# alexfrom0815/IR-BPP

Hardware: AMD Instinct MI355X
Metric: env steps/sec (placements/sec) across N parallel bins (higher is better)
Workload: dtype f64

## Files before the change

irbpp_amd/build.py:

```python
from __future__ import annotations

import os
import shutil
import subprocess

PKG_DIR = os.path.dirname(os.path.abspath(__file__))
CSRC = os.path.join(PKG_DIR, "csrc")
LIB_PATH = os.path.join(PKG_DIR, "libirbpp_hip.so")
SOURCES = ["irbpp_capi.hip", "irbpp_kernels.hip", "irbpp_wide.hip", "irbpp_replay.hip", "irbpp_replay_pool.hip", "irbpp_metrics.hip", "irbpp_metrics.h", "irbpp_device.h", "contours_device.h", "irbpp_itemgen.h",
           "irbpp_itemgen.hip", "irbpp_itemgen_device.h", "irbpp_rotalias.h", "irbpp_head.h", "irbpp_c51.hip", "irbpp_dueling.hip", "irbpp_dueling_loss.hip", "irbpp_streams.hip", "irbpp_plan.h", "irbpp_binstate.h", "irbpp_binstate.hip",
           os.path.join("..", "..", "include", "irbpp.h")]
HIPCC_FLAGS = ["--offload-arch=gfx950", "-O3", "-std=c++17", "-ffp-contract=off", "-fno-honor-nans",
               "-shared", "-fPIC", "-Wno-unused-value"]


def source_hash() -> str:
    import hashlib
    h = hashlib.sha256(" ".join(HIPCC_FLAGS).encode())
    for name in sorted(SOURCES):
        with open(os.path.join(CSRC, name), "rb") as f:
            h.update(f.read())
    return h.hexdigest()[:16]


def _hipcc() -> str:
    for cand in (shutil.which("hipcc"), "/opt/rocm/bin/hipcc"):
        if cand and os.path.exists(cand):
            return cand
    raise RuntimeError("hipcc not found: the HIP library cannot be built on this machine")


def built_hash(path: str = LIB_PATH) -> str:
    try:
        with open(path, "rb") as f:
            blob = f.read()
    except OSError:
        return ""
    i = blob.find(b"irbpp-source-hash:")
    return blob[i + 18:i + 34].decode("ascii", "replace") if i >= 0 else ""


def needs_build(path: str = LIB_PATH) -> bool:
    return built_hash(path) != source_hash()


def build(force: bool = False, verbose: bool = False) -> str:
    out = LIB_PATH
    if not force and not needs_build(out):
        return out
    cmd = [_hipcc()] + HIPCC_FLAGS + [f'-DIRBPP_SOURCE_HASH="{source_hash()}"', os.path.join(CSRC, "irbpp_capi.hip"), "-o", out]
    if verbose:
        print(" ".join(cmd))
    res = subprocess.run(cmd, capture_output=True, text=True)
    if res.returncode != 0:
        raise RuntimeError("hipcc failed:\n" + res.stdout + res.stderr)
    from . import asmcheck
    try:
        chk = asmcheck.check_library(out)
    except (RuntimeError, OSError, subprocess.CalledProcessError) as e:
        if verbose:
            print(f"asmcheck skipped: {e}")
        return out
    if verbose:
        print(f"asmcheck: {chk['scalar_loads']} scalar loads in {chk['functions']} kernels, {len(chk['problems'])} hazards")
    if chk["problems"]:
        os.replace(out, out + ".rejected")
        raise RuntimeError("scalar-load hazard in the built library (kept as " + out + ".rejected):\n" + "\n".join(chk["problems"]))
    return out
```

irbpp_amd/csrc/irbpp_kernels.hip:

```cpp
#include <hip/hip_runtime.h>
#include <math.h>
#include <stdint.h>

#include "contours_device.h"
#include "irbpp_device.h"
#include "../../include/irbpp.h"

#ifndef IRBPP_PASS
#define IRBPP_PASS 1
#endif

#undef IRBPP_HERE
#undef IRBPP_PASS_NS
#if IRBPP_PASS == 1
#define IRBPP_HERE ::irbpp::
#elif IRBPP_PASS == 2
#define IRBPP_HERE ::irbpp::wg512::
#define IRBPP_PASS_NS wg512
#else
#define IRBPP_HERE ::irbpp::wg128::
#define IRBPP_PASS_NS wg128
#endif

namespace irbpp {
#if IRBPP_PASS != 1
namespace IRBPP_PASS_NS {
#endif

#if IRBPP_PASS == 1
constexpr int BLOCK = 256;
#elif IRBPP_PASS == 2
constexpr int BLOCK = 512;
#else
constexpr int BLOCK = 128;
#endif
constexpr int WAVES = BLOCK / 64;

#ifndef IRBPP_REPS
#ifdef IRBPP_ABLATE
#define IRBPP_REPS(bit) (1 + ((P.dbg_repeat >> (bit)) & 1))
#else
#define IRBPP_REPS(bit) 1
#endif
#endif

#if IRBPP_PASS == 1
__device__ __forceinline__ double round6(double x) { return rint(x * 1e6) / 1e6; }

__device__ __forceinline__ double round6_scaled(double x) { return rint(x * 1e6); }

__device__ __forceinline__ int np_floor_divide_int(double a, double b, double inv_b) {
    const double x = fabs(a);
    const double q0 = trunc(x * inv_b);
    const double r0 = fma(-q0, b, x);
    int q = (int)q0 + (r0 >= b ? 1 : 0) - (r0 < 0.0 ? 1 : 0);
#if defined(__HIP_DEVICE_COMPILE__)
    if (__ballot(a < 0.0) == 0ull) return q;
#endif
    if (a < 0.0) {
        const double r = fma(-(double)q, b, x);
        q = r == 0.0 ? -q : -q - 1;
    }
    return q;
}

template <int CTRL, int ROW_MASK>
__device__ __forceinline__ int dpp_shift(int v) { return __builtin_amdgcn_update_dpp(0, v, CTRL, ROW_MASK, 0xF, false); }
__device__ __forceinline__ int wave_inclusive_sum(int v) {
    v += dpp_shift<0x111, 0xF>(v);
    v += dpp_shift<0x112, 0xF>(v);
    v += dpp_shift<0x114, 0xF>(v);
    v += dpp_shift<0x118, 0xF>(v);
    v += dpp_shift<0x142, 0xA>(v);
    v += dpp_shift<0x143, 0xC>(v);
    return v;
}
__device__ __forceinline__ int imax(int a, int b) { return a > b ? a : b; }
__device__ __forceinline__ int wave_inclusive_max(int v) {
    v = imax(v, dpp_shift<0x111, 0xF>(v));
    v = imax(v, dpp_shift<0x112, 0xF>(v));
    v = imax(v, dpp_shift<0x114, 0xF>(v));
    v = imax(v, dpp_shift<0x118, 0xF>(v));
    v = imax(v, dpp_shift<0x142, 0xA>(v));
    v = imax(v, dpp_shift<0x143, 0xC>(v));
    return v;
}

__device__ __forceinline__ double wave_max_f64(double v) {
#define IRBPP_MAX_STEP(CTRL, ROWS)                                                                                   \
    {                                                                                                                \
        const int lo = __builtin_amdgcn_update_dpp(__double2loint(v), __double2loint(v), CTRL, ROWS, 0xF, false);    \
        const int hi = __builtin_amdgcn_update_dpp(__double2hiint(v), __double2hiint(v), CTRL, ROWS, 0xF, false);    \
        v = fmax(v, __hiloint2double(hi, lo));                                                                       \
    }
    IRBPP_MAX_STEP(0x111, 0xF) IRBPP_MAX_STEP(0x112, 0xF) IRBPP_MAX_STEP(0x114, 0xF) IRBPP_MAX_STEP(0x118, 0xF)
    IRBPP_MAX_STEP(0x142, 0xA) IRBPP_MAX_STEP(0x143, 0xC)
#undef IRBPP_MAX_STEP
    return __hiloint2double(__builtin_amdgcn_readlane(__double2hiint(v), 63), __builtin_amdgcn_readlane(__double2loint(v), 63));
}

#endif
__device__ inline double block_max_f64(double v, double* red) {
    v = wave_max_f64(v);
    __syncthreads();
    if ((threadIdx.x & 63) == 0) red[threadIdx.x >> 6] = v;
    __syncthreads();
    double r = red[0];
    for (int w = 1; w < WAVES; ++w) r = fmax(r, red[w]);
    return r;
}

__device__ inline int block_sum_int(int v, int* red) {
    v = __builtin_amdgcn_readlane(wave_inclusive_sum(v), 63);
    __syncthreads();
    if ((threadIdx.x & 63) == 0) red[threadIdx.x >> 6] = v;
    __syncthreads();
    int r = 0;
    for (int w = 0; w < WAVES; ++w) r += red[w];
    return r;
}

__device__ inline int block_scan_flag(bool flag, int* red, int& total) {
    const unsigned long long bal = __ballot(flag);
    const int lane = threadIdx.x & 63, w = threadIdx.x >> 6;
    const int pre = __popcll(bal & ((1ull << lane) - 1ull));
    __syncthreads();
    if (lane == 0) red[w] = __popcll(bal);
    __syncthreads();
    int base = 0;
    total = 0;
    for (int i = 0; i < WAVES; ++i) {
        const int c = red[i];
        if (i < w) base += c;
        total += c;
    }
    return base + pre;
}

#if IRBPP_PASS == 1
__device__ inline int trajectory_row(const Params& P, const Tables& T, int b, int episode) {
    long long row = T.stream ? (long long)b : (long long)P.traj_start + P.goff + b + (long long)episode * P.gbins;
    row %= T.n_traj;
    if (row < 0) row += T.n_traj;
    return (int)row;
}
struct KernArgs;
__device__ __forceinline__ void raise_error(const State& S, int bit);
constexpr int STREAM_CONSUMED = -3;
__device__ inline int consume_item(const Tables& T, const State& S, int row, int cursor, int id) {
    if (T.stream) {
        if (id == STREAM_CONSUMED) { raise_error(S, IRBPP_DEVERR_STREAM_DRY); return -1; }
        const_cast<int32_t*>(T.seq)[(long long)row * T.seq_len + (int)((uint32_t)cursor % (uint32_t)T.seq_len)] = STREAM_CONSUMED;
    }
    if (id >= T.n_shapes) { raise_error(S, IRBPP_DEVERR_BAD_ITEM); return -1; }
    return id < 0 ? -1 : id;
}
__device__ inline int fetch_item(const Tables& T, const State& S, int row, int cursor) {
    if (!T.stream && cursor >= T.seq_len) return -1;
    const int at = T.stream ? (int)((uint32_t)cursor % (uint32_t)T.seq_len) : cursor;
    return consume_item(T, S, row, cursor, T.seq[(long long)row * T.seq_len + at]);
}

__device__ __forceinline__ int fdiv(int n, int d, uint32_t m) {
    return d == 1 ? n : (int)__umulhi((uint32_t)n, m);
}

struct KernArgs { Params P; Tables T; State S; StepIO io; int mode; };
typedef const __attribute__((address_space(4))) KernArgs* KernArgsPtr;
__device__ __forceinline__ KernArgsPtr cold_args() {
// ... 1496 lines not shown
                    } else {
                        k = keys[row];
                    }
                    float rv;
                    if (fallback) rv = (float)((gvalid[(k >> 16) * 16 + ((k >> 8) & 255u)] >> (k & 255u)) & 1u);
                    else rv = (float)zsrc[(k >> 16) * AC + ((k >> 8) & 255u) * Ay + (k & 255u)];
                    v0 = (float)(k >> 16);
                    v1 = (float)((k >> 8) & 255u);
                    v2 = (float)(k & 255u);
                    v3 = fallback ? (float)P.bin_z : rv;
                    v4 = fallback ? rv : 1.0f;
                    S.cand[(size_t)b * P.S + row] = k;
                    if (!fallback && rv < best) { best = rv; bi = row; }
                }
                float* const o = obs + 5 * row;
                o[0] = v0; o[1] = v1; o[2] = v2; o[3] = v3; o[4] = v4;
            }
            if (lane == 0) {
                S.bs[b].cur_item = item;
                S.bs[b].nvalid = nvalid;
                S.bs[b].nrows = nrows;
            }
            if (io.auto_action != nullptr) {
#define IRBPP_ARGMIN_STEP(CTRL, ROWS)                                                                                          \
                {                                                                                                              \
                    const float ob = __int_as_float(__builtin_amdgcn_update_dpp(__float_as_int(best), __float_as_int(best), CTRL, ROWS, 0xF, false)); \
                    const int oi = __builtin_amdgcn_update_dpp(bi, bi, CTRL, ROWS, 0xF, false);                                 \
                    if (ob < best || (ob == best && oi < bi)) { best = ob; bi = oi; }                                           \
                }
                IRBPP_ARGMIN_STEP(0x111, 0xF) IRBPP_ARGMIN_STEP(0x112, 0xF) IRBPP_ARGMIN_STEP(0x114, 0xF) IRBPP_ARGMIN_STEP(0x118, 0xF)
                IRBPP_ARGMIN_STEP(0x142, 0xA) IRBPP_ARGMIN_STEP(0x143, 0xC)
#undef IRBPP_ARGMIN_STEP
                if (lane == 63) io.auto_action[b] = bi == 0x7fffffff ? 0 : bi;
            }
            stamp(io, b, 4, lane == 0);
        }
    }
    __syncthreads();
    if ((need[0] & need[1] & need[2] & need[3]) == -1) return;
    Lds L = {};
    L.vmask = (uint32_t*)(smem + P.e_vmask);
    L.redd = (double*)(smem + P.e_red);
    L.redi = (int*)(L.redd + 8);
    L.img = (uint16_t*)(smem + P.e_hist);
    L.scratch = smem + P.e_keys;
#pragma unroll 1
    for (int w = 0; w < WAVES; ++w) {
        const int bw = __builtin_amdgcn_readfirstlane(need[w]);
        if (bw < 0) continue;
        const int slot_w = (int)blockIdx.x * WAVES + w + io.block_off;
        float* const obs = io.obs + (size_t)(some ? slot_w : bw) * io.obs_stride;
        const uint32_t* gv = S.w_vmask + (size_t)bw * R * 16;
        __syncthreads();
#pragma unroll 1
        for (int i = tid; i < R * 16; i += BLOCK) L.vmask[i] = gv[i];
        const int nvalid = S.w_meta[(size_t)bw * WMETA + 2], item = S.w_meta[(size_t)bw * WMETA + 3];
        const uint32_t amap_w = (uint32_t)S.w_meta[(size_t)bw * WMETA + 5];
        __syncthreads();
        stamp(io, bw, 3);
        emit_observation(P, S, io, L, bw, item, nvalid, obs, S.w_posz + (size_t)bw * R * AC, S.w_valid + (size_t)bw * R * 16, amap_w);
    }
}
#define IRBPP_EMIT_WAVE_KERNEL(NAME, SPEC)                                                                                  \
    extern "C" __global__ void __launch_bounds__(BLOCK) __attribute__((amdgpu_waves_per_eu(8, 8)))                      \
    NAME(const Params P, const Tables T, const State S, const StepIO io, const int mode) {                              \
        extern __shared__ __attribute__((aligned(16))) unsigned char smem[];                                            \
        emit_wave_body<SPEC>(P, T, S, io, mode, smem);                                                                  \
    }
IRBPP_EMIT_WAVE_KERNEL(irbpp_emit_wave_kernel, 0)
#ifndef IRBPP_NO_SPEC
IRBPP_EMIT_WAVE_KERNEL(irbpp_emit_wave_kernel_s1, 1)
IRBPP_EMIT_WAVE_KERNEL(irbpp_emit_wave_kernel_s2, 2)
IRBPP_EMIT_WAVE_KERNEL(irbpp_emit_wave_kernel_s5, 5)
#endif

#ifndef IRBPP_TRACE_SHORT
#define IRBPP_TRACE_SHORT 0
#endif
constexpr int TRACE_P = IRBPP_TRACE_P;
constexpr int TRACE_CAP = 128;
constexpr int TRACE_LDS_CAP = 56, TRACE_SLOT = TRACE_LDS_CAP + 4;
constexpr int TRACE_SPILL = TRACE_CAP - TRACE_LDS_CAP;
constexpr int TRACE_SHORT = IRBPP_TRACE_SHORT;
static_assert(TRACE_CAP <= 64 * TRACE_P, "a border must fit one polygon round");
static_assert(ROUND_POINTS == 64 * TRACE_P, "a round record holds one polygon round");
constexpr int TRACE_BIG = 768;
constexpr int TRACE_FSTRIDE = FRAME_WORDS;
static_assert(TRACE_FSTRIDE % 2 == 1 && (TRACE_SLOT / 4) % 2 == 1 && TRACE_SLOT % 4 == 0, "odd dword strides in LDS");
constexpr int TRACE_BIG_BYTES = 6 * TRACE_BIG + 64;
constexpr int TRACE_WAVE_BYTES = TRACE_BIG_BYTES + 64 * TRACE_SPILL;
template <int TRACE_CPW>
__device__ __forceinline__ void trace_body(const Params& P, const State& S, long long* prof) {
    constexpr int SLOT = TRACE_SLOT, CAP = TRACE_CAP, LCAP = TRACE_LDS_CAP, PP = TRACE_P;
    __shared__ __attribute__((aligned(16))) uint8_t slots[TRACE_CPW * SLOT];
    __shared__ __attribute__((aligned(16))) uint32_t sfr[TRACE_CPW * TRACE_FSTRIDE];
    __shared__ uint32_t dps[64 * PP];
    __shared__ uint8_t dpscratch[64 * PP];
    const int lane = threadIdx.x;
    const int seg_cap = P.seg_cap;
    int seg_n[NXCD], seg_first[NXCD + 1];
    seg_first[0] = 0;
#pragma unroll
    for (int s = 0; s < NXCD; ++s) {
        const int n = S.w_total[s * XCD_STRIDE];
        seg_n[s] = n < seg_cap ? n : seg_cap;
        seg_first[s + 1] = seg_first[s] + (seg_n[s] + TRACE_CPW - 1) / TRACE_CPW;
    }
    for (int chunk = blockIdx.x; chunk < seg_first[NXCD]; chunk += gridDim.x) {
        const long long t_start = prof ? (long long)clock64() : 0;
        int seg = 0;
#pragma unroll
        for (int s = 1; s < NXCD; ++s) seg += chunk >= seg_first[s] ? 1 : 0;
        int first_chunk = 0, count = 0;
#pragma unroll
        for (int s = 0; s < NXCD; ++s) if (s == seg) { first_chunk = seg_first[s]; count = seg_n[s]; }
        const int gi = (chunk - first_chunk) * TRACE_CPW + lane;
        const bool have = lane < TRACE_CPW && gi < count;
        const size_t g = (size_t)seg * seg_cap + gi;
        int my_n = 0, rk = 0, x0 = 0, y0 = 0;
        uint32_t* const fr = sfr + (lane < TRACE_CPW ? lane : 0) * TRACE_FSTRIDE;
        uint8_t* const my_slot = slots + (lane < TRACE_CPW ? lane : 0) * SLOT;
        uint8_t* const wave_spill = S.w_big + (size_t)blockIdx.x * TRACE_WAVE_BYTES + TRACE_BIG_BYTES;
        if (have) {
            const uint2 ce = S.w_cand[g];
            const uint32_t e = ce.y;
            const int b = (int)ce.x, img = (int)((e >> 8) & 511u);
            x0 = e & 15u;
            y0 = (e >> 4) & 15u;
            rk = b * P.R + (int)S.w_imgrot[(size_t)b * P.wimg + img];
            const uint4* gi = (const uint4*)(S.w_img + ((size_t)b * P.wimg + img) * 16);
            const uint4 v0 = gi[0], v1 = gi[1];
            const uint32_t w[8] = {v0.x, v0.y, v0.z, v0.w, v1.x, v1.y, v1.z, v1.w};
            uint32_t r[16], c[16];
#pragma unroll
            for (int q = 0; q < 8; ++q) {
                r[2 * q] = c[2 * q] = w[q] & 0xFFFFu;
                r[2 * q + 1] = c[2 * q + 1] = w[q] >> 16;
            }
            transpose16(c);
            frames_store(fr, r, c);
        }
        const long long t_staged = prof ? (long long)clock64() : 0;
        {
            const int n = trace_border_fast(fr, x0, y0, my_slot, LCAP, have, wave_spill + lane * TRACE_SPILL, TRACE_SPILL);
            if (n < 0) { if (lane == 0) atomicOr(S.err, IRBPP_DEVERR_TRACE_GUARD); }
            else my_n = n;
        }
        {
            unsigned long long big = __ballot(my_n > CAP);
            while (big != 0ull) {
                const int l0 = __ffsll((long long)big) - 1;
                big &= big - 1ull;
                if (lane == l0) {
                    uint8_t* gsc = S.w_big + (size_t)blockIdx.x * TRACE_WAVE_BYTES;
                    SlotMem m;
                    m.pts = gsc; m.dst = gsc + TRACE_BIG; m.stk = (uint32_t*)(gsc + 2 * TRACE_BIG); m.cap = TRACE_BIG; m.cap_stk = TRACE_BIG;
                    uint16_t* im = (uint16_t*)(gsc + 6 * TRACE_BIG);
                    for (int q = 0; q < 16; ++q) { im[q] = (uint16_t)frame_raw_row(fr, q); im[16 + q] = (uint16_t)frame_raw_col(fr, q); }
                    if (contour_vertices(im, im + 16, x0, y0, m, S.w_vmask + (size_t)rk * 16) != 0)
                        atomicOr(S.err, IRBPP_DEVERR_TRACE_GUARD);
                    my_n = 0;
                }
            }
        }
        const bool spilled = __ballot(my_n > LCAP) != 0ull;
        if (spilled) {
            __builtin_amdgcn_fence(__ATOMIC_RELEASE, "workgroup");
            __builtin_amdgcn_fence(__ATOMIC_ACQUIRE, "workgroup");
        }
        const long long t_traced = prof ? (long long)clock64() : 0;
        auto next_round = [&](int cls, int left, int& wn, int& excl, int& base) -> unsigned long long {
            wn = (cls == 0 ? left <= TRACE_SHORT : true) ? left : 0;
            const int incl = wave_inclusive_sum(wn);
            excl = incl - wn;
            if (__builtin_amdgcn_readlane(incl, 63) == 0) return 0ull;
            const unsigned long long todo = __ballot(wn > 0);
            base = __builtin_amdgcn_readlane(excl, __ffsll((long long)todo) - 1);
            return __ballot(wn > 0 && incl - base <= 64 * PP);
        };
        int n_rounds = 0;
        {
            int left = my_n;
            for (int cls = 0; cls < 2; ++cls)
                for (;;) {
                    int wn, excl, base = 0;
                    const unsigned long long sel = next_round(cls, left, wn, excl, base);
                    if (sel == 0ull) break;
                    if ((sel >> lane) & 1ull) left = 0;
                    ++n_rounds;
                }
        }
        const int round_cap = P.round_cap;
        const int xcd = (int)(__builtin_amdgcn_s_getreg((31 << 11) | 20) & (NXCD - 1));
        int at = 0;
        if (n_rounds > 0) {
            if (lane == 0) at = atomicAdd(S.w_nround + xcd * XCD_STRIDE, n_rounds);
            at = __builtin_amdgcn_readfirstlane(at);
        }
        const bool inline_dp = at + n_rounds > round_cap;
        uint8_t* const rec0 = S.w_round + ((size_t)xcd * round_cap + at) * ROUND_BYTES;
        int left = my_n, n_dp = 0;
        for (int cls = 0; cls < 2; ++cls)
        for (;;) {
            int wn, excl, base = 0;
            const unsigned long long sel = next_round(cls, left, wn, excl, base);
            if (sel == 0ull) break;
#pragma unroll
            for (int u = 0; u < PP; ++u) dps[u * 64 + lane] = 0u;
            IRBPP_WAVE_SYNC();
            if ((sel >> lane) & 1ull) dps[excl - base] = (uint32_t)lane + 1u;
            IRBPP_WAVE_SYNC();
            int mark[PP];
#pragma unroll
            for (int u = 0; u < PP; ++u) mark[u] = (int)dps[u * 64 + lane];
            IRBPP_WAVE_SYNC();
            bool live[PP];
            int pv[PP], jj[PP], nn[PP], sbq[PP], prk[PP];
            const uint8_t* pts[PP];
            int carry = 0;
#pragma unroll
            for (int u = 0; u < PP; ++u) {
                const int run = imax(wave_inclusive_max(mark[u]), carry);
                carry = __builtin_amdgcn_readlane(run, 63);
                const int owner = run - 1;
                const int on = owner >= 0 ? owner : 0;
                const int ns = __shfl(wn | ((excl - base) << 8), on);
                nn[u] = ns & 255;
                sbq[u] = ns >> 8;
                prk[u] = __shfl(rk, on);
                live[u] = owner >= 0 && u * 64 + lane < sbq[u] + nn[u];
                pts[u] = slots + on * SLOT;
                jj[u] = u * 64 + lane - sbq[u];
                if (!live[u]) { nn[u] = 1; sbq[u] = 0; jj[u] = 0; }
                pv[u] = live[u] ? (int)pts[u][jj[u] < LCAP ? jj[u] : LCAP] : 0;
                if (spilled && live[u] && jj[u] >= LCAP) pv[u] = (int)wave_spill[on * TRACE_SPILL + jj[u] - LCAP];
            }
            if (inline_dp) {
                approx_convex_segmented<PP>(lane, live, pv, jj, nn, sbq, pts, prk, dps, dpscratch, S.w_vmask);
            } else {
                uint8_t* const rec = rec0 + (size_t)n_dp * ROUND_BYTES;
#pragma unroll
                for (int u = 0; u < PP; ++u) {
                    const int q = u * 64 + lane;
                    rec[q] = (uint8_t)pv[u];
                    rec[64 * PP + q] = (uint8_t)(live[u] ? nn[u] : 0);
                    rec[2 * 64 * PP + q] = (uint8_t)sbq[u];
                    ((uint32_t*)(rec + 3 * 64 * PP))[q] = (uint32_t)prk[u];
                }
            }
            if ((sel >> lane) & 1ull) left = 0;
            ++n_dp;
        }
        if (inline_dp && n_rounds > 0 && at < round_cap) {
            const int lim = at + n_rounds < round_cap ? n_rounds : round_cap - at;
            for (int i = 0; i < lim; ++i)
#pragma unroll
                for (int u = 0; u < PP; ++u) rec0[(size_t)i * ROUND_BYTES + 64 * PP + u * 64 + lane] = 0;
        }
#if defined(IRBPP_AB_POLY_ACCOUNT) || defined(IRBPP_AB_EMIT_ACCOUNT)
        if (false) {
#else
        if (prof && lane == 0) {
#endif
            const int b0 = (int)S.w_cand[(size_t)seg * seg_cap + (size_t)(chunk - first_chunk) * TRACE_CPW].x;
            long long* row = prof + (size_t)b0 * PHASE_ROW;
            const long long t_end = (long long)clock64();
            row[11] = t_end - t_start;
            row[12] = t_staged - t_start;
            row[13] = t_traced - t_staged;
            row[14] = t_end - t_traced;
            row[15] = 1 | ((long long)n_dp << 20) | ((long long)(count - (chunk - first_chunk) * TRACE_CPW < TRACE_CPW ? count - (chunk - first_chunk) * TRACE_CPW : TRACE_CPW) << 40);
        }
        IRBPP_WAVE_SYNC();
    }
}

constexpr int TRACE_REFILL_BATCH = 128, TRACE_REFILL_THR = 32;
template <int BATCH, int THR>
__device__ __forceinline__ void trace_refill_body(const Params& P, const State& S, long long* prof) {
    constexpr int SLOT = TRACE_SLOT, CAP = TRACE_CAP, LCAP = TRACE_LDS_CAP, PP = TRACE_P, NCE = BATCH / 64;
    static_assert(BATCH % 64 == 0 && NCE >= 1 && NCE <= 4, "a batch is a whole number of wave-wide candidate loads");
    __shared__ __attribute__((aligned(16))) uint8_t slots[64 * SLOT];
    __shared__ __attribute__((aligned(16))) uint32_t sfr[64 * TRACE_FSTRIDE];
    __shared__ uint32_t dps[64 * PP];
    __shared__ uint8_t dpscratch[64 * PP];
    const int lane = threadIdx.x;
    const int seg_cap = P.seg_cap;
    int seg_n[NXCD], seg_first[NXCD + 1];
    seg_first[0] = 0;
#pragma unroll
    for (int s = 0; s < NXCD; ++s) {
        const int n = S.w_total[s * XCD_STRIDE];
        seg_n[s] = n < seg_cap ? n : seg_cap;
        seg_first[s + 1] = seg_first[s] + (seg_n[s] + BATCH - 1) / BATCH;
    }
    uint32_t* const fr = sfr + lane * TRACE_FSTRIDE;
    uint8_t* const my_slot = slots + lane * SLOT;
    uint8_t* const wave_spill = S.w_big + (size_t)blockIdx.x * TRACE_WAVE_BYTES + TRACE_BIG_BYTES;
    uint8_t* const my_spill = wave_spill + lane * TRACE_SPILL;
    IRBPP_WALK_TABLES(WT)
    const int round_cap = P.round_cap;
    const int xcd = (int)(__builtin_amdgcn_s_getreg((31 << 11) | 20) & (NXCD - 1));
    for (int chunk = blockIdx.x; chunk < seg_first[NXCD]; chunk += gridDim.x) {
        const long long t_start = prof ? (long long)clock64() : 0;
        int seg = 0;
#pragma unroll
        for (int s = 1; s < NXCD; ++s) seg += chunk >= seg_first[s] ? 1 : 0;
        int first_chunk = 0, count = 0;
#pragma unroll
        for (int s = 0; s < NXCD; ++s) if (s == seg) { first_chunk = seg_first[s]; count = seg_n[s]; }
        const int gi0 = (chunk - first_chunk) * BATCH;
        const int nb = count - gi0 < BATCH ? count - gi0 : BATCH;
        const uint2* const cl = S.w_cand + (size_t)seg * seg_cap + gi0;
        uint2 ce[NCE];
#pragma unroll
        for (int u = 0; u < NCE; ++u) ce[u] = u * 64 + lane < nb ? cl[u * 64 + lane] : make_uint2(0u, 0u);
        Walk w;
        w.pos = w.n = w.result = w.pos0 = w.pos1 = 0;
        w.nb16 = w.k2 = w.prev = w.s_close = w.run = 0u;
        int rk = 0, x0 = 0, y0 = 0, nxt = 0, n_dp_total = 0, refills = 0;
        uint2 pf_e = make_uint2(0u, 0u);
        uint4 pf0 = make_uint4(0u, 0u, 0u, 0u), pf1 = pf0;
        uint32_t pf_rot = 0u;
        auto prefetch = [&]() {
            const int c = nxt + lane;
            uint2 e = make_uint2(0u, 0u);
#pragma unroll
            for (int u = 0; u < NCE; ++u) {
                const uint32_t ex = (uint32_t)__shfl((int)ce[u].x, c & 63), ey = (uint32_t)__shfl((int)ce[u].y, c & 63);
                if ((c >> 6) == u) e = make_uint2(ex, ey);
            }
            pf_e = e;
            if (c < nb) {
                const size_t at = (size_t)e.x * P.wimg + ((e.y >> 8) & 511u);
                pf_rot = S.w_imgrot[at];
                const uint4* gi = (const uint4*)(S.w_img + at * 16);
                pf0 = gi[0];
                pf1 = gi[1];
            }
        };
        auto flush = [&]() {
            int my_n = w.run == 0u ? w.result : 0;
            w.result = w.run == 0u ? 0 : w.result;
            if (__ballot(my_n != 0) == 0ull) return;
            {
                unsigned long long big = __ballot(my_n > CAP);
                while (big != 0ull) {
                    const int l0 = __ffsll((long long)big) - 1;
                    big &= big - 1ull;
                    if (lane == l0) {
                        uint8_t* gsc = S.w_big + (size_t)blockIdx.x * TRACE_WAVE_BYTES;
                        SlotMem m;
                        m.pts = gsc; m.dst = gsc + TRACE_BIG; m.stk = (uint32_t*)(gsc + 2 * TRACE_BIG); m.cap = TRACE_BIG; m.cap_stk = TRACE_BIG;
                        uint16_t* im = (uint16_t*)(gsc + 6 * TRACE_BIG);
                        for (int q = 0; q < 16; ++q) { im[q] = (uint16_t)frame_raw_row(fr, q); im[16 + q] = (uint16_t)frame_raw_col(fr, q); }
                        if (contour_vertices(im, im + 16, x0, y0, m, S.w_vmask + (size_t)rk * 16) != 0)
                            atomicOr(S.err, IRBPP_DEVERR_TRACE_GUARD);
                        my_n = 0;
                    }
                }
            }
            const bool spilled = __ballot(my_n > LCAP) != 0ull;
            if (spilled) {
                __builtin_amdgcn_fence(__ATOMIC_RELEASE, "workgroup");
                __builtin_amdgcn_fence(__ATOMIC_ACQUIRE, "workgroup");
            }
            auto next_round = [&](int left, int& wn, int& excl, int& base) -> unsigned long long {
                wn = left;
                const int incl = wave_inclusive_sum(wn);
                excl = incl - wn;
                if (__builtin_amdgcn_readlane(incl, 63) == 0) return 0ull;
                const unsigned long long todo = __ballot(wn > 0);
                base = __builtin_amdgcn_readlane(excl, __ffsll((long long)todo) - 1);
                return __ballot(wn > 0 && incl - base <= 64 * PP);
            };
            int n_rounds = 0;
            {
                int left = my_n;
                for (;;) {
                    int wn, excl, base = 0;
                    const unsigned long long sel = next_round(left, wn, excl, base);
                    if (sel == 0ull) break;
                    if ((sel >> lane) & 1ull) left = 0;
                    ++n_rounds;
                }
            }
            int at = 0;
            if (n_rounds > 0) {
                if (lane == 0) at = atomicAdd(S.w_nround + xcd * XCD_STRIDE, n_rounds);
                at = __builtin_amdgcn_readfirstlane(at);
            }
            const bool inline_dp = at + n_rounds > round_cap;
            uint8_t* const rec0 = S.w_round + ((size_t)xcd * round_cap + at) * ROUND_BYTES;
            int left = my_n, n_dp = 0;
            for (;;) {
                int wn, excl, base = 0;
                const unsigned long long sel = next_round(left, wn, excl, base);
                if (sel == 0ull) break;
#pragma unroll
                for (int u = 0; u < PP; ++u) dps[u * 64 + lane] = 0u;
                IRBPP_WAVE_SYNC();
                if ((sel >> lane) & 1ull) dps[excl - base] = (uint32_t)lane + 1u;
                IRBPP_WAVE_SYNC();
                int mark[PP];
#pragma unroll
                for (int u = 0; u < PP; ++u) mark[u] = (int)dps[u * 64 + lane];
                IRBPP_WAVE_SYNC();
                bool live[PP];
                int pv[PP], jj[PP], nn[PP], sbq[PP], prk[PP];
                const uint8_t* pts[PP];
                int carry = 0;
#pragma unroll
                for (int u = 0; u < PP; ++u) {
                    const int run = imax(wave_inclusive_max(mark[u]), carry);
                    carry = __builtin_amdgcn_readlane(run, 63);
                    const int owner = run - 1;
                    const int on = owner >= 0 ? owner : 0;
                    const int ns = __shfl(wn | ((excl - base) << 8), on);
                    nn[u] = ns & 255;
                    sbq[u] = ns >> 8;
                    prk[u] = __shfl(rk, on);
                    live[u] = owner >= 0 && u * 64 + lane < sbq[u] + nn[u];
                    pts[u] = slots + on * SLOT;
                    jj[u] = u * 64 + lane - sbq[u];
                    if (!live[u]) { nn[u] = 1; sbq[u] = 0; jj[u] = 0; }
                    pv[u] = live[u] ? (int)pts[u][jj[u] < LCAP ? jj[u] : LCAP] : 0;
                    if (spilled && live[u] && jj[u] >= LCAP) pv[u] = (int)wave_spill[on * TRACE_SPILL + jj[u] - LCAP];
                }
                if (inline_dp) {
                    approx_convex_segmented<PP>(lane, live, pv, jj, nn, sbq, pts, prk, dps, dpscratch, S.w_vmask);
                } else {
                    uint8_t* const rec = rec0 + (size_t)n_dp * ROUND_BYTES;
#pragma unroll
                    for (int u = 0; u < PP; ++u) {
                        const int q = u * 64 + lane;
                        rec[q] = (uint8_t)pv[u];
                        rec[64 * PP + q] = (uint8_t)(live[u] ? nn[u] : 0);
                        rec[2 * 64 * PP + q] = (uint8_t)sbq[u];
                        ((uint32_t*)(rec + 3 * 64 * PP))[q] = (uint32_t)prk[u];
                    }
                }
                if ((sel >> lane) & 1ull) left = 0;
                ++n_dp;
            }
            if (inline_dp && n_rounds > 0 && at < round_cap) {
                const int lim = at + n_rounds < round_cap ? n_rounds : round_cap - at;
                for (int i = 0; i < lim; ++i)
#pragma unroll
                    for (int u = 0; u < PP; ++u) rec0[(size_t)i * ROUND_BYTES + 64 * PP + u * 64 + lane] = 0;
            }
            n_dp_total += n_dp;
            IRBPP_WAVE_SYNC();
        };
        prefetch();
        int guard = 16384;
        for (;;) {
            const unsigned long long walking = __ballot(w.run != 0u);
            const int idle = 64 - __popcll(walking);
            if ((idle >= THR && nxt < nb) || walking == 0ull) {
                flush();
                if (nxt >= nb) break;
                const int rank = (int)__builtin_amdgcn_mbcnt_hi((uint32_t)(~walking >> 32), __builtin_amdgcn_mbcnt_lo((uint32_t)~walking, 0u));
                const bool take = w.run == 0u && nxt + rank < nb;
                const uint32_t ex = (uint32_t)__shfl((int)pf_e.x, rank), ey = (uint32_t)__shfl((int)pf_e.y, rank);
                const uint32_t rot = (uint32_t)__shfl((int)pf_rot, rank);
                uint32_t wd[8];
                wd[0] = (uint32_t)__shfl((int)pf0.x, rank); wd[1] = (uint32_t)__shfl((int)pf0.y, rank);
                wd[2] = (uint32_t)__shfl((int)pf0.z, rank); wd[3] = (uint32_t)__shfl((int)pf0.w, rank);
                wd[4] = (uint32_t)__shfl((int)pf1.x, rank); wd[5] = (uint32_t)__shfl((int)pf1.y, rank);
                wd[6] = (uint32_t)__shfl((int)pf1.z, rank); wd[7] = (uint32_t)__shfl((int)pf1.w, rank);
                if (take) {
                    x0 = (int)(ey & 15u);
                    y0 = (int)((ey >> 4) & 15u);
                    rk = (int)ex * P.R + (int)rot;
                    uint32_t r[16], c[16];
#pragma unroll
                    for (int q = 0; q < 8; ++q) {
                        r[2 * q] = c[2 * q] = wd[q] & 0xFFFFu;
                        r[2 * q + 1] = c[2 * q + 1] = wd[q] >> 16;
                    }
                    transpose16(c);
                    frames_store(fr, r, c);
                    walk_start(w, fr, x0, y0, my_slot, LCAP, true, WT);
                }
                nxt += idle < nb - nxt ? idle : nb - nxt;
                ++refills;
                if (nxt < nb) prefetch();
                continue;
            }
            if (w.run != 0u) walk_iter(w, fr, my_slot, LCAP, my_spill, TRACE_SPILL, WT);
            if (--guard == 0) { if (lane == 0) atomicOr(S.err, IRBPP_DEVERR_TRACE_GUARD); break; }
        }
        if (prof && lane == 0) {
            const int b0 = (int)cl[0].x;
            long long* row = prof + (size_t)b0 * PHASE_ROW;
            const long long t_end = (long long)clock64();
            row[11] = t_end - t_start;
            row[12] = 0;
            row[13] = t_end - t_start;
            row[14] = (long long)refills | ((long long)(16384 - guard) << 16);
            row[15] = 1 | ((long long)n_dp_total << 20) | ((long long)nb << 40);
        }
        IRBPP_WAVE_SYNC();
    }
}
extern "C" __global__ void __launch_bounds__(64) irbpp_trace_kernel_refill(const Params P, const State S, long long* prof) {
    trace_refill_body<TRACE_REFILL_BATCH, TRACE_REFILL_THR>(P, S, prof);
}

extern "C" __global__ void __launch_bounds__(64) irbpp_trace_kernel(const Params P, const State S, long long* prof) { trace_body<64>(P, S, prof); }
extern "C" __global__ void __launch_bounds__(64) irbpp_trace_kernel_c32(const Params P, const State S, long long* prof) { trace_body<32>(P, S, prof); }
extern "C" __global__ void __launch_bounds__(64) irbpp_trace_kernel_c16(const Params P, const State S, long long* prof) { trace_body<16>(P, S, prof); }

extern "C" __global__ void __launch_bounds__(64)
irbpp_polygon_kernel(const Params P, const State S
#ifdef IRBPP_AB_POLY_ACCOUNT
                     , long long* prof
#endif
                     ) {
    constexpr int PP = TRACE_P;
#ifdef IRBPP_AB_POLY_ACCOUNT
    long long acct[8] = {0, 0, 0, 0, 0, 0, 0, 0};
    long long* const ac = prof ? acct : nullptr;
    const long long t_begin = (long long)clock64(), w_begin = (long long)wall_clock64();
    long long t_first_loaded = 0, cyc_hops = 0, cyc_dp = 0, cyc_rank = 0, cyc_tail = 0, rounds_done = 0;
#endif
    __shared__ uint32_t dps[64 * PP];
    __shared__ uint8_t dpscratch[64 * PP];
    __shared__ __attribute__((aligned(16))) uint8_t lpts[64 * PP];
    const int lane = threadIdx.x;
    const int round_cap = P.round_cap;
    int seg_n[NXCD], seg_first[NXCD + 1];
    seg_first[0] = 0;
#pragma unroll
    for (int s = 0; s < NXCD; ++s) {
        const int n = S.w_nround[s * XCD_STRIDE];
        seg_n[s] = n < round_cap ? n : round_cap;
        seg_first[s + 1] = seg_first[s] + seg_n[s];
    }
    for (int rd = blockIdx.x; rd < seg_first[NXCD]; rd += gridDim.x) {
        int seg = 0;
#pragma unroll
        for (int s = 1; s < NXCD; ++s) seg += rd >= seg_first[s] ? 1 : 0;
        int first = 0;
#pragma unroll
        for (int s = 0; s < NXCD; ++s) if (s == seg) first = seg_first[s];
        const uint8_t* const rec = S.w_round + ((size_t)seg * round_cap + (rd - first)) * ROUND_BYTES;
        bool live[PP];
        int pv[PP], jj[PP], nn[PP], sbq[PP], prk[PP];
        const uint8_t* pts[PP];
#pragma unroll
        for (int u = 0; u < PP; ++u) {
            const int q = u * 64 + lane;
            pv[u] = rec[q];
            nn[u] = rec[64 * PP + q];
            sbq[u] = rec[2 * 64 * PP + q];
            prk[u] = (int)((const uint32_t*)(rec + 3 * 64 * PP))[q];
            lpts[q] = (uint8_t)pv[u];
        }
        IRBPP_WAVE_SYNC();
#pragma unroll
        for (int u = 0; u < PP; ++u) {
            live[u] = nn[u] > 0;
            jj[u] = u * 64 + lane - sbq[u];
            if (!live[u]) { nn[u] = 1; sbq[u] = 0; jj[u] = 0; pv[u] = 0; }
            pts[u] = lpts + sbq[u];
        }
#ifdef IRBPP_AB_POLY_ACCOUNT
        const long long t_in = (long long)clock64();
        if (rounds_done == 0) t_first_loaded = t_in - t_begin;
        acct[1] = acct[2] = acct[3] = 0;
        approx_convex_segmented<PP>(lane, live, pv, jj, nn, sbq, pts, prk, dps, dpscratch, S.w_vmask, ac);
        const long long t_out = (long long)clock64();
        cyc_hops += acct[1] - t_in; cyc_dp += acct[2] - acct[1]; cyc_rank += acct[3] - acct[2]; cyc_tail += t_out - acct[3];
        ++rounds_done;
#else
        approx_convex_segmented<PP>(lane, live, pv, jj, nn, sbq, pts, prk, dps, dpscratch, S.w_vmask);
#endif
        IRBPP_WAVE_SYNC();
    }
#ifdef IRBPP_AB_POLY_ACCOUNT
    if (prof && lane == 0 && (int)blockIdx.x < P.N) {
        long long* row = prof + (size_t)blockIdx.x * PHASE_ROW;
        row[11] = (long long)clock64() - t_begin;
        row[12] = t_first_loaded | (((long long)(__builtin_amdgcn_s_getreg((31 << 11) | 20) & (NXCD - 1))) << 32);
        row[10] = w_begin;
        row[9] = (long long)wall_clock64();
        row[13] = cyc_hops | (cyc_dp << 32);
        row[14] = cyc_rank | (cyc_tail << 32);
        row[15] = rounds_done | (acct[5] << 8) | (acct[6] << 24);
    }
#endif
}

#endif
template <int PATH, int SPEC, bool FUSED, bool CHAIN = false>
__device__ __forceinline__ void env_transition(const Params& P_run, const Tables& T, const State& S, const StepIO& io,
                                               const int mode, unsigned char* smem);

#if IRBPP_PASS == 1
#ifndef IRBPP_ENV_WAVES
#define IRBPP_ENV_WAVES 8
#endif
#define IRBPP_ENV_KERNEL(NAME, PATH, SPEC, ATTR)                                                                        \
    extern "C" __global__ void __launch_bounds__(BLOCK) ATTR                                                           \
    NAME(const Params P, const Tables T, const State S, const StepIO io, const int mode) {                             \
        extern __shared__ __attribute__((aligned(16))) unsigned char smem[];                                           \
        env_transition<PATH, SPEC, true>(P, T, S, io, mode, smem);                                                     \
    }
#define IRBPP_CAPPED __attribute__((amdgpu_waves_per_eu(IRBPP_ENV_WAVES, IRBPP_ENV_WAVES)))
IRBPP_ENV_KERNEL(irbpp_env_kernel, PATH_BLOCK, 0, IRBPP_CAPPED)
IRBPP_ENV_KERNEL(irbpp_env_kernel_box8, PATH_BOX, 0, IRBPP_CAPPED)
IRBPP_ENV_KERNEL(irbpp_env_kernel_box, PATH_BOX, 0, )
IRBPP_ENV_KERNEL(irbpp_env_kernel_generic8, PATH_GENERIC, 0, IRBPP_CAPPED)
IRBPP_ENV_KERNEL(irbpp_env_kernel_generic, PATH_GENERIC, 0, )
IRBPP_ENV_KERNEL(irbpp_env_kernel_wide, PATH_ANY, 0, )
IRBPP_ENV_KERNEL(irbpp_env_kernel_mixed8, PATH_MIXED, 0, IRBPP_CAPPED)
#define IRBPP_ENV_KERNEL_CHAIN(NAME, PATH, SPEC)                                                                        \
    extern "C" __global__ void __launch_bounds__(BLOCK)                                                                \
    NAME(const Params P, const Tables T, const State S, const StepIO io, const int mode) {                             \
        extern __shared__ __attribute__((aligned(16))) unsigned char smem[];                                           \
        env_transition<PATH, SPEC, true, true>(P, T, S, io, mode, smem);                                               \
    }
IRBPP_ENV_KERNEL_CHAIN(irbpp_env_kernel_chain, PATH_ANY, 0)
#ifndef IRBPP_NO_SPEC
IRBPP_ENV_KERNEL(irbpp_env_kernel_s1, PATH_BLOCK, 1, IRBPP_CAPPED)
IRBPP_ENV_KERNEL(irbpp_env_kernel_s2, PATH_BOX, 2, IRBPP_CAPPED)
IRBPP_ENV_KERNEL(irbpp_env_kernel_s3, PATH_GENERIC, 3, IRBPP_CAPPED)
IRBPP_ENV_KERNEL(irbpp_env_kernel_s4, PATH_GENERIC, 4, )
IRBPP_ENV_KERNEL(irbpp_env_kernel_s5, PATH_MIXED, 5, IRBPP_CAPPED)
IRBPP_ENV_KERNEL_CHAIN(irbpp_env_kernel_chain_s1, PATH_BLOCK, 1)
#endif

#elif IRBPP_PASS == 3
extern "C" __global__ void __launch_bounds__(128)
irbpp_env_kernel_s1_w128(const Params P, const Tables T, const State S, const StepIO io, const int mode) {
    extern __shared__ __attribute__((aligned(16))) unsigned char smem[];
    IRBPP_HERE env_transition<PATH_BLOCK, 1, true>(P, T, S, io, mode, smem);
}
#else
#define IRBPP_ENV_KERNEL_512(NAME, PATH, SPEC, ATTR)                                                                    \
    extern "C" __global__ void __launch_bounds__(512) ATTR                                                             \
    NAME(const Params P, const Tables T, const State S, const StepIO io, const int mode) {                             \
        extern __shared__ __attribute__((aligned(16))) unsigned char smem[];                                           \
        IRBPP_HERE env_transition<PATH, SPEC, true>(P, T, S, io, mode, smem);                                          \
    }
IRBPP_ENV_KERNEL_512(irbpp_env_kernel_generic_w512, PATH_GENERIC, 0, )
#ifndef IRBPP_NO_SPEC
IRBPP_ENV_KERNEL_512(irbpp_env_kernel_s4_w512, PATH_GENERIC, 4, )
IRBPP_ENV_KERNEL_512(irbpp_env_kernel_s4_w512c, PATH_GENERIC, 4, __attribute__((amdgpu_waves_per_eu(8, 8))))
#endif
#endif

template <int PATH, int SPEC, bool FUSED, bool CHAIN>
__device__ __forceinline__ void env_transition(const Params& P_run, const Tables& T, const State& S, const StepIO& io,
                                               const int mode, unsigned char* smem) {
    if constexpr (!FUSED) { if (mode == MODE_STEP) return; }
    Params P_spec;
    const Params& P = SPEC == 0 ? P_run : (P_spec = specialise<SPEC>(P_run), P_spec);
    const Lds L = carve_lds(smem, P);
// ... 820 lines not shown
```

Measured before the change: 68.66 million.

## Merge short and long borders into fewer polygon rounds and skip empty halves

Moves round packing into a shared helper with a merge policy: after the short-border class is fully selected, long borders that still fit the remaining round capacity join the same round, which reduces the number of DP rounds. The convex-approximation call checks whether the second half of a round is empty across the wave and then runs the single-width variant, and the polygon kernel skips LDS writes for empty halves. The polygon kernel is also pinned to 8 waves per EU. The cost is extra wave scans per round selection and a register cap that could cause spills.

```diff
diff --git a/irbpp_amd/build.py b/irbpp_amd/build.py
--- a/irbpp_amd/build.py
+++ b/irbpp_amd/build.py
@@ -8,7 +8,7 @@
 CSRC = os.path.join(PKG_DIR, "csrc")
 LIB_PATH = os.path.join(PKG_DIR, "libirbpp_hip.so")
 SOURCES = ["irbpp_capi.hip", "irbpp_kernels.hip", "irbpp_wide.hip", "irbpp_replay.hip", "irbpp_replay_pool.hip", "irbpp_metrics.hip", "irbpp_metrics.h", "irbpp_device.h", "contours_device.h", "irbpp_itemgen.h",
-           "irbpp_itemgen.hip", "irbpp_itemgen_device.h", "irbpp_rotalias.h", "irbpp_head.h", "irbpp_c51.hip", "irbpp_dueling.hip", "irbpp_dueling_loss.hip", "irbpp_streams.hip", "irbpp_plan.h", "irbpp_binstate.h", "irbpp_binstate.hip",
+           "irbpp_itemgen.hip", "irbpp_itemgen_device.h", "irbpp_rotalias.h", "irbpp_head.h", "irbpp_c51.hip", "irbpp_dueling.hip", "irbpp_dueling_loss.hip", "irbpp_streams.hip", "irbpp_plan.h", "irbpp_binstate.h", "irbpp_binstate.hip", "irbpp_round_packing.h",
            os.path.join("..", "..", "include", "irbpp.h")]
 HIPCC_FLAGS = ["--offload-arch=gfx950", "-O3", "-std=c++17", "-ffp-contract=off", "-fno-honor-nans",
                "-shared", "-fPIC", "-Wno-unused-value"]
diff --git a/irbpp_amd/csrc/irbpp_kernels.hip b/irbpp_amd/csrc/irbpp_kernels.hip
--- a/irbpp_amd/csrc/irbpp_kernels.hip
+++ b/irbpp_amd/csrc/irbpp_kernels.hip
@@ -4,6 +4,7 @@
 
 #include "contours_device.h"
 #include "irbpp_device.h"
+#include "irbpp_round_packing.h"
 #include "../../include/irbpp.h"
 
 #ifndef IRBPP_PASS
@@ -64,27 +65,6 @@
     return q;
 }
 
-template <int CTRL, int ROW_MASK>
-__device__ __forceinline__ int dpp_shift(int v) { return __builtin_amdgcn_update_dpp(0, v, CTRL, ROW_MASK, 0xF, false); }
-__device__ __forceinline__ int wave_inclusive_sum(int v) {
-    v += dpp_shift<0x111, 0xF>(v);
-    v += dpp_shift<0x112, 0xF>(v);
-    v += dpp_shift<0x114, 0xF>(v);
-    v += dpp_shift<0x118, 0xF>(v);
-    v += dpp_shift<0x142, 0xA>(v);
-    v += dpp_shift<0x143, 0xC>(v);
-    return v;
-}
-__device__ __forceinline__ int imax(int a, int b) { return a > b ? a : b; }
-__device__ __forceinline__ int wave_inclusive_max(int v) {
-    v = imax(v, dpp_shift<0x111, 0xF>(v));
-    v = imax(v, dpp_shift<0x112, 0xF>(v));
-    v = imax(v, dpp_shift<0x114, 0xF>(v));
-    v = imax(v, dpp_shift<0x118, 0xF>(v));
-    v = imax(v, dpp_shift<0x142, 0xA>(v));
-    v = imax(v, dpp_shift<0x143, 0xC>(v));
-    return v;
-}
 
 __device__ __forceinline__ double wave_max_f64(double v) {
 #define IRBPP_MAX_STEP(CTRL, ROWS)                                                                                   \
@@ -1747,6 +1727,7 @@
 constexpr int TRACE_LDS_CAP = 56, TRACE_SLOT = TRACE_LDS_CAP + 4;
 constexpr int TRACE_SPILL = TRACE_CAP - TRACE_LDS_CAP;
 constexpr int TRACE_SHORT = IRBPP_TRACE_SHORT;
+constexpr int TRACE_PACK = PACK_MERGE;
 static_assert(TRACE_CAP <= 64 * TRACE_P, "a border must fit one polygon round");
 static_assert(ROUND_POINTS == 64 * TRACE_P, "a round record holds one polygon round");
 constexpr int TRACE_BIG = 768;
@@ -1754,6 +1735,20 @@
 static_assert(TRACE_FSTRIDE % 2 == 1 && (TRACE_SLOT / 4) % 2 == 1 && TRACE_SLOT % 4 == 0, "odd dword strides in LDS");
 constexpr int TRACE_BIG_BYTES = 6 * TRACE_BIG + 64;
 constexpr int TRACE_WAVE_BYTES = TRACE_BIG_BYTES + 64 * TRACE_SPILL;
+__device__ __forceinline__ void approx_convex_round(int lane, const bool (&live)[TRACE_P], const int (&pv)[TRACE_P], const int (&j)[TRACE_P],
+                                                    const int (&n)[TRACE_P], const int (&sb)[TRACE_P], const uint8_t* const (&pts)[TRACE_P],
+                                                    const int (&rot)[TRACE_P], uint32_t* slots, uint8_t* scratch, uint32_t* vmask) {
+    static_assert(TRACE_P == 2, "the half-width round is the first of two words of positions");
+    if (__ballot(live[1]) == 0ull) {
+        const bool live1[1] = {live[0]};
+        const int pv1[1] = {pv[0]}, j1[1] = {j[0]}, n1[1] = {n[0]}, sb1[1] = {sb[0]}, rot1[1] = {rot[0]};
+        const uint8_t* const pts1[1] = {pts[0]};
+        approx_convex_segmented<1>(lane, live1, pv1, j1, n1, sb1, pts1, rot1, slots, scratch, vmask);
+    } else {
+        approx_convex_segmented<TRACE_P>(lane, live, pv, j, n, sb, pts, rot, slots, scratch, vmask);
+    }
+}
+
 template <int TRACE_CPW>
 __device__ __forceinline__ void trace_body(const Params& P, const State& S, long long* prof) {
     constexpr int SLOT = TRACE_SLOT, CAP = TRACE_CAP, LCAP = TRACE_LDS_CAP, PP = TRACE_P;
@@ -1834,27 +1829,7 @@
             __builtin_amdgcn_fence(__ATOMIC_ACQUIRE, "workgroup");
         }
         const long long t_traced = prof ? (long long)clock64() : 0;
-        auto next_round = [&](int cls, int left, int& wn, int& excl, int& base) -> unsigned long long {
-            wn = (cls == 0 ? left <= TRACE_SHORT : true) ? left : 0;
-            const int incl = wave_inclusive_sum(wn);
-            excl = incl - wn;
-            if (__builtin_amdgcn_readlane(incl, 63) == 0) return 0ull;
-            const unsigned long long todo = __ballot(wn > 0);
-            base = __builtin_amdgcn_readlane(excl, __ffsll((long long)todo) - 1);
-            return __ballot(wn > 0 && incl - base <= 64 * PP);
-        };
-        int n_rounds = 0;
-        {
-            int left = my_n;
-            for (int cls = 0; cls < 2; ++cls)
-                for (;;) {
-                    int wn, excl, base = 0;
-                    const unsigned long long sel = next_round(cls, left, wn, excl, base);
-                    if (sel == 0ull) break;
-                    if ((sel >> lane) & 1ull) left = 0;
-                    ++n_rounds;
-                }
-        }
+        const int n_rounds = pack_rounds<64 * PP, TRACE_SHORT, TRACE_PACK>(lane, my_n, [](int, unsigned long long, int, int) {});
         const int round_cap = P.round_cap;
         const int xcd = (int)(__builtin_amdgcn_s_getreg((31 << 11) | 20) & (NXCD - 1));
         int at = 0;
@@ -1864,16 +1839,11 @@
         }
         const bool inline_dp = at + n_rounds > round_cap;
         uint8_t* const rec0 = S.w_round + ((size_t)xcd * round_cap + at) * ROUND_BYTES;
-        int left = my_n, n_dp = 0;
-        for (int cls = 0; cls < 2; ++cls)
-        for (;;) {
-            int wn, excl, base = 0;
-            const unsigned long long sel = next_round(cls, left, wn, excl, base);
-            if (sel == 0ull) break;
+        const int n_dp = pack_rounds<64 * PP, TRACE_SHORT, TRACE_PACK>(lane, my_n, [&](int k, unsigned long long sel, int wn, int start) {
 #pragma unroll
             for (int u = 0; u < PP; ++u) dps[u * 64 + lane] = 0u;
             IRBPP_WAVE_SYNC();
-            if ((sel >> lane) & 1ull) dps[excl - base] = (uint32_t)lane + 1u;
+            if ((sel >> lane) & 1ull) dps[start] = (uint32_t)lane + 1u;
             IRBPP_WAVE_SYNC();
             int mark[PP];
 #pragma unroll
@@ -1889,7 +1859,7 @@
                 carry = __builtin_amdgcn_readlane(run, 63);
                 const int owner = run - 1;
                 const int on = owner >= 0 ? owner : 0;
-                const int ns = __shfl(wn | ((excl - base) << 8), on);
+                const int ns = __shfl(wn | (start << 8), on);
                 nn[u] = ns & 255;
                 sbq[u] = ns >> 8;
                 prk[u] = __shfl(rk, on);
@@ -1901,9 +1871,9 @@
                 if (spilled && live[u] && jj[u] >= LCAP) pv[u] = (int)wave_spill[on * TRACE_SPILL + jj[u] - LCAP];
             }
             if (inline_dp) {
-                approx_convex_segmented<PP>(lane, live, pv, jj, nn, sbq, pts, prk, dps, dpscratch, S.w_vmask);
+                approx_convex_round(lane, live, pv, jj, nn, sbq, pts, prk, dps, dpscratch, S.w_vmask);
             } else {
-                uint8_t* const rec = rec0 + (size_t)n_dp * ROUND_BYTES;
+                uint8_t* const rec = rec0 + (size_t)k * ROUND_BYTES;
 #pragma unroll
                 for (int u = 0; u < PP; ++u) {
                     const int q = u * 64 + lane;
@@ -1913,9 +1883,7 @@
                     ((uint32_t*)(rec + 3 * 64 * PP))[q] = (uint32_t)prk[u];
                 }
             }
-            if ((sel >> lane) & 1ull) left = 0;
-            ++n_dp;
-        }
+        });
         if (inline_dp && n_rounds > 0 && at < round_cap) {
             const int lim = at + n_rounds < round_cap ? n_rounds : round_cap - at;
             for (int i = 0; i < lim; ++i)
@@ -2030,26 +1998,7 @@
                 __builtin_amdgcn_fence(__ATOMIC_RELEASE, "workgroup");
                 __builtin_amdgcn_fence(__ATOMIC_ACQUIRE, "workgroup");
             }
-            auto next_round = [&](int left, int& wn, int& excl, int& base) -> unsigned long long {
-                wn = left;
-                const int incl = wave_inclusive_sum(wn);
-                excl = incl - wn;
-                if (__builtin_amdgcn_readlane(incl, 63) == 0) return 0ull;
-                const unsigned long long todo = __ballot(wn > 0);
-                base = __builtin_amdgcn_readlane(excl, __ffsll((long long)todo) - 1);
-                return __ballot(wn > 0 && incl - base <= 64 * PP);
-            };
-            int n_rounds = 0;
-            {
-                int left = my_n;
-                for (;;) {
-                    int wn, excl, base = 0;
-                    const unsigned long long sel = next_round(left, wn, excl, base);
-                    if (sel == 0ull) break;
-                    if ((sel >> lane) & 1ull) left = 0;
-                    ++n_rounds;
-                }
-            }
+            const int n_rounds = pack_rounds<64 * PP, 0, TRACE_PACK>(lane, my_n, [](int, unsigned long long, int, int) {});
             int at = 0;
             if (n_rounds > 0) {
                 if (lane == 0) at = atomicAdd(S.w_nround + xcd * XCD_STRIDE, n_rounds);
@@ -2057,15 +2006,11 @@
             }
             const bool inline_dp = at + n_rounds > round_cap;
             uint8_t* const rec0 = S.w_round + ((size_t)xcd * round_cap + at) * ROUND_BYTES;
-            int left = my_n, n_dp = 0;
-            for (;;) {
-                int wn, excl, base = 0;
-                const unsigned long long sel = next_round(left, wn, excl, base);
-                if (sel == 0ull) break;
+            const int n_dp = pack_rounds<64 * PP, 0, TRACE_PACK>(lane, my_n, [&](int k, unsigned long long sel, int wn, int start) {
 #pragma unroll
                 for (int u = 0; u < PP; ++u) dps[u * 64 + lane] = 0u;
                 IRBPP_WAVE_SYNC();
-                if ((sel >> lane) & 1ull) dps[excl - base] = (uint32_t)lane + 1u;
+                if ((sel >> lane) & 1ull) dps[start] = (uint32_t)lane + 1u;
                 IRBPP_WAVE_SYNC();
                 int mark[PP];
 #pragma unroll
@@ -2081,7 +2026,7 @@
                     carry = __builtin_amdgcn_readlane(run, 63);
                     const int owner = run - 1;
                     const int on = owner >= 0 ? owner : 0;
-                    const int ns = __shfl(wn | ((excl - base) << 8), on);
+                    const int ns = __shfl(wn | (start << 8), on);
                     nn[u] = ns & 255;
                     sbq[u] = ns >> 8;
                     prk[u] = __shfl(rk, on);
@@ -2093,9 +2038,9 @@
                     if (spilled && live[u] && jj[u] >= LCAP) pv[u] = (int)wave_spill[on * TRACE_SPILL + jj[u] - LCAP];
                 }
                 if (inline_dp) {
-                    approx_convex_segmented<PP>(lane, live, pv, jj, nn, sbq, pts, prk, dps, dpscratch, S.w_vmask);
+                    approx_convex_round(lane, live, pv, jj, nn, sbq, pts, prk, dps, dpscratch, S.w_vmask);
                 } else {
-                    uint8_t* const rec = rec0 + (size_t)n_dp * ROUND_BYTES;
+                    uint8_t* const rec = rec0 + (size_t)k * ROUND_BYTES;
 #pragma unroll
                     for (int u = 0; u < PP; ++u) {
                         const int q = u * 64 + lane;
@@ -2105,9 +2050,7 @@
                         ((uint32_t*)(rec + 3 * 64 * PP))[q] = (uint32_t)prk[u];
                     }
                 }
-                if ((sel >> lane) & 1ull) left = 0;
-                ++n_dp;
-            }
+            });
             if (inline_dp && n_rounds > 0 && at < round_cap) {
                 const int lim = at + n_rounds < round_cap ? n_rounds : round_cap - at;
                 for (int i = 0; i < lim; ++i)
@@ -2177,7 +2120,7 @@
 extern "C" __global__ void __launch_bounds__(64) irbpp_trace_kernel_c32(const Params P, const State S, long long* prof) { trace_body<32>(P, S, prof); }
 extern "C" __global__ void __launch_bounds__(64) irbpp_trace_kernel_c16(const Params P, const State S, long long* prof) { trace_body<16>(P, S, prof); }
 
-extern "C" __global__ void __launch_bounds__(64)
+extern "C" __global__ void __launch_bounds__(64) __attribute__((amdgpu_waves_per_eu(8, 8)))
 irbpp_polygon_kernel(const Params P, const State S
 #ifdef IRBPP_AB_POLY_ACCOUNT
                      , long long* prof
@@ -2221,7 +2164,7 @@
             nn[u] = rec[64 * PP + q];
             sbq[u] = rec[2 * 64 * PP + q];
             prk[u] = (int)((const uint32_t*)(rec + 3 * 64 * PP))[q];
-            lpts[q] = (uint8_t)pv[u];
+            if (u == 0 || __ballot(nn[u] > 0) != 0ull) lpts[q] = (uint8_t)pv[u];
         }
         IRBPP_WAVE_SYNC();
 #pragma unroll
@@ -2240,7 +2183,7 @@
         cyc_hops += acct[1] - t_in; cyc_dp += acct[2] - acct[1]; cyc_rank += acct[3] - acct[2]; cyc_tail += t_out - acct[3];
         ++rounds_done;
 #else
-        approx_convex_segmented<PP>(lane, live, pv, jj, nn, sbq, pts, prk, dps, dpscratch, S.w_vmask);
+        approx_convex_round(lane, live, pv, jj, nn, sbq, pts, prk, dps, dpscratch, S.w_vmask);
 #endif
         IRBPP_WAVE_SYNC();
     }
diff --git a/irbpp_amd/csrc/irbpp_round_packing.h b/irbpp_amd/csrc/irbpp_round_packing.h
--- /dev/null
+++ b/irbpp_amd/csrc/irbpp_round_packing.h
@@ -0,0 +1,80 @@
+#pragma once
+
+namespace irbpp {
+
+#ifndef IRBPP_HOST_WAVE
+template <int CTRL, int ROW_MASK>
+__device__ __forceinline__ int dpp_shift(int v) { return __builtin_amdgcn_update_dpp(0, v, CTRL, ROW_MASK, 0xF, false); }
+__device__ __forceinline__ int wave_inclusive_sum(int v) {
+    v += dpp_shift<0x111, 0xF>(v);
+    v += dpp_shift<0x112, 0xF>(v);
+    v += dpp_shift<0x114, 0xF>(v);
+    v += dpp_shift<0x118, 0xF>(v);
+    v += dpp_shift<0x142, 0xA>(v);
+    v += dpp_shift<0x143, 0xC>(v);
+    return v;
+}
+__device__ __forceinline__ int imax(int a, int b) { return a > b ? a : b; }
+__device__ __forceinline__ int wave_inclusive_max(int v) {
+    v = imax(v, dpp_shift<0x111, 0xF>(v));
+    v = imax(v, dpp_shift<0x112, 0xF>(v));
+    v = imax(v, dpp_shift<0x114, 0xF>(v));
+    v = imax(v, dpp_shift<0x118, 0xF>(v));
+    v = imax(v, dpp_shift<0x142, 0xA>(v));
+    v = imax(v, dpp_shift<0x143, 0xC>(v));
+    return v;
+}
+#endif
+
+constexpr int PACK_NEXT_FIT = 0, PACK_MERGE = 1, PACK_FILL = 2;
+
+template <int POINTS, int SHORT, int ORDER>
+__device__ __forceinline__ unsigned long long round_select(int lane, int cls, int left, int& wn, int& start) {
+    const bool mine = SHORT > 0 && cls == 0 ? left <= SHORT : true;
+    wn = mine ? left : 0;
+    const int incl = wave_inclusive_sum(wn);
+    const int excl = incl - wn;
+    start = 0;
+    if (__builtin_amdgcn_readlane(incl, 63) == 0) return 0ull;
+    const unsigned long long todo = __ballot(wn > 0);
+    const int base = __builtin_amdgcn_readlane(excl, __ffsll((long long)todo) - 1);
+    unsigned long long sel = __ballot(wn > 0 && incl - base <= POINTS);
+    start = excl - base;
+    if (ORDER == PACK_NEXT_FIT) return sel;
+    const int used = __builtin_amdgcn_readlane(incl, 63 - __clzll((long long)sel)) - base;
+    if (ORDER == PACK_FILL && sel != todo) {
+        const int w2 = (wn > 0 && !((sel >> lane) & 1ull) && wn <= POINTS - used) ? wn : 0;
+        const int incl2 = wave_inclusive_sum(w2);
+        const unsigned long long sel2 = __ballot(w2 > 0 && incl2 <= POINTS - used);
+        if ((sel2 >> lane) & 1ull) start = used + incl2 - w2;
+        return sel | sel2;
+    }
+    if (SHORT > 0 && cls == 0 && sel == todo) {
+        const int w1 = left > SHORT ? left : 0;
+        const int incl1 = wave_inclusive_sum(w1);
+        const unsigned long long sel1 = __ballot(w1 > 0 && incl1 <= POINTS - used);
+        if (sel1 == 0ull) return sel;
+        sel |= sel1;
+        wn = (sel >> lane) & 1ull ? left : 0;
+        const int inclm = wave_inclusive_sum(wn);
+        start = inclm - wn;
+    }
+    return sel;
+}
+
+template <int POINTS, int SHORT, int ORDER, class F>
+__device__ __forceinline__ int pack_rounds(int lane, int my_n, F&& on_round) {
+    int left = my_n, k = 0;
+    for (int cls = SHORT > 0 ? 0 : 1; cls < 2; ++cls)
+        for (;;) {
+            int wn, start;
+            const unsigned long long sel = round_select<POINTS, SHORT, ORDER>(lane, cls, left, wn, start);
+            if (sel == 0ull) break;
+            on_round(k, sel, wn, start);
+            if ((sel >> lane) & 1ull) left = 0;
+            ++k;
+        }
+    return k;
+}
+
+}
```

Result: no change. 69.62 million, median of 6 (+1.4%).
